# BichenWuUCB/squeezeDet

Hardware: NVIDIA H100
Metric: images/sec (1242x375, b=20) (higher is better)
Workload: dtype f32 (3xTF32 wgmma, fp32 accumulate)

## Files before the change

squeezedet_b200/csrc/conv_pool_simt.cu:

```cuda
#include <math_constants.h>

#include "common.cuh"

namespace sqdet {
namespace {

constexpr int PT_H = 4, PT_W = 16;
constexpr int CT_H = 2 * PT_H + 1, CT_W = 2 * PT_W + 1;
constexpr int CT_PIX = CT_H * CT_W;
constexpr int PIX_PER_THREAD = (CT_PIX + 63) / 64;

struct ConvPoolParams {
  const float* x;
  const float* w;
  const float* bias;
  const float* scale;
  const float* shift;
  float* y;
  int B, H, W, Cout;
  int Hc, Wc;
  int Hp, Wp;
  int cpad_t, cpad_l;
  int ppad_t, ppad_l;
  int relu;
  int tiles_w, tiles_h;
};

template <int KS, int NT, int MINB>
__global__ void __launch_bounds__(NT, MINB)
conv_pool_simt_kernel(const ConvPoolParams p) {
  constexpr int PH = 2 * (CT_H - 1) + KS;
  constexpr int PW = 2 * (CT_W - 1) + KS;
  constexpr int K = KS * KS * 3;
  extern __shared__ __align__(16) float sm[];
  float* s_patch = sm;
  float* s_w = s_patch + ((PH * PW * 3 + 3) & ~3);
  float* s_conv = s_w + K * p.Cout;

  const int tid = threadIdx.x;
  const int nthreads = blockDim.x;
  int tile = blockIdx.x;
  const int tw = tile % p.tiles_w;
  tile /= p.tiles_w;
  const int th = tile % p.tiles_h;
  const int img = tile / p.tiles_h;
  const int ph0 = th * PT_H, pw0 = tw * PT_W;
  const int ch0 = 2 * ph0 - p.ppad_t, cw0 = 2 * pw0 - p.ppad_l;
  const int iy0 = 2 * ch0 - p.cpad_t, ix0 = 2 * cw0 - p.cpad_l;

  for (int i = tid; i < K * p.Cout / 4; i += nthreads) {
    const unsigned dst = (unsigned)__cvta_generic_to_shared(s_w + i * 4);
    asm volatile("cp.async.cg.shared.global [%0], [%1], 16;" ::"r"(dst), "l"(p.w + i * 4) : "memory");
  }
  {
    const float* xin = p.x + (size_t)img * p.H * p.W * 3;
    const int wid = tid >> 5, lane = tid & 31, nwarps = nthreads >> 5;
    for (int row = wid; row < PH; row += nwarps) {
      const int iy = iy0 + row;
      const bool row_ok = iy >= 0 && iy < p.H;
      const float* src = xin + (size_t)(row_ok ? iy : 0) * p.W * 3;
#pragma unroll
      for (int it = 0; it < (PW * 3 + 31) / 32; ++it) {
        const int col = lane + it * 32;
        if (col < PW * 3) {
          const int ixc = ix0 * 3 + col;
          const bool ok = row_ok && ixc >= 0 && ixc < p.W * 3;
          const unsigned dst = (unsigned)__cvta_generic_to_shared(s_patch + row * (PW * 3) + col);
          const int nbytes = ok ? 4 : 0;
          asm volatile("cp.async.ca.shared.global [%0], [%1], 4, %2;" ::"r"(dst),
                       "l"(src + (ok ? ixc : 0)), "r"(nbytes)
                       : "memory");
        }
      }
    }
  }
  asm volatile("cp.async.commit_group;" ::: "memory");
  asm volatile("cp.async.wait_group 0;" ::: "memory");
  __syncthreads();

  const int cg = tid >> 6;
  const int l64 = tid & 63;
  float acc[PIX_PER_THREAD][16];
#pragma unroll
  for (int i = 0; i < PIX_PER_THREAD; ++i)
#pragma unroll
    for (int c = 0; c < 16; ++c) acc[i][c] = 0.f;
  int pbase[PIX_PER_THREAD];
#pragma unroll
  for (int i = 0; i < PIX_PER_THREAD; ++i) {
    int px = l64 + 64 * i;
    if (px >= CT_PIX) px = CT_PIX - 1;
    const int cr = px / CT_W, cc = px - cr * CT_W;
    pbase[i] = (2 * cr * PW + 2 * cc) * 3;
  }
  const float* wg = s_w + cg * 16;
  for (int a = 0; a < KS; ++a) {
#pragma unroll
    for (int bc = 0; bc < KS * 3; ++bc) {
      const int k = a * KS * 3 + bc;
      float xx[PIX_PER_THREAD];
#pragma unroll
      for (int i = 0; i < PIX_PER_THREAD; ++i) xx[i] = s_patch[pbase[i] + a * PW * 3 + bc];
#pragma unroll
      for (int q = 0; q < 4; ++q) {
        const float4 w4 = *reinterpret_cast<const float4*>(wg + k * p.Cout + q * 4);
        const float wv[4] = {w4.x, w4.y, w4.z, w4.w};
#pragma unroll
        for (int i = 0; i < PIX_PER_THREAD; ++i)
#pragma unroll
          for (int c = 0; c < 4; ++c) acc[i][q * 4 + c] = fmaf(xx[i], wv[c], acc[i][q * 4 + c]);
      }
    }
  }

  {
    float bv[16], sv[16], hv[16];
#pragma unroll
    for (int c = 0; c < 16; ++c) {
      bv[c] = p.bias ? __ldg(p.bias + cg * 16 + c) : 0.f;
      sv[c] = p.scale ? __ldg(p.scale + cg * 16 + c) : 1.f;
      hv[c] = p.scale ? __ldg(p.shift + cg * 16 + c) : 0.f;
    }
    float* tile_c = s_conv + (size_t)cg * CT_PIX * 16;
#pragma unroll
    for (int i = 0; i < PIX_PER_THREAD; ++i) {
      const int px = l64 + 64 * i;
      if (px < CT_PIX) {
        const int cr = px / CT_W, cc = px - cr * CT_W;
        const int oh = ch0 + cr, ow = cw0 + cc;
        const bool ok = oh >= 0 && oh < p.Hc && ow >= 0 && ow < p.Wc;
        const int sw = (px >> 1) & 3;
#pragma unroll
        for (int j = 0; j < 4; ++j) {
          float o[4];
#pragma unroll
          for (int e = 0; e < 4; ++e) {
            float f = acc[i][j * 4 + e] + bv[j * 4 + e];
            if (p.scale) f = f * sv[j * 4 + e] + hv[j * 4 + e];
            if (p.relu) f = fmaxf(f, 0.f);
            o[e] = ok ? f : -CUDART_INF_F;
          }
          *reinterpret_cast<float4*>(tile_c + px * 16 + ((j ^ sw) << 2)) =
              make_float4(o[0], o[1], o[2], o[3]);
        }
      }
    }
  }
  __syncthreads();

  const int chunks = p.Cout / 4;
  for (int u = tid; u < PT_H * PT_W * chunks; u += nthreads) {
    const int chunk = u % chunks, pp = u / chunks;
    const int py = pp / PT_W, pxp = pp - py * PT_W;
    const int ph = ph0 + py, pw = pw0 + pxp;
    if (ph >= p.Hp || pw >= p.Wp) continue;
    const int g = chunk >> 2, j = chunk & 3;
    const float* tile_c = s_conv + (size_t)g * CT_PIX * 16;
    float4 m = make_float4(-CUDART_INF_F, -CUDART_INF_F, -CUDART_INF_F, -CUDART_INF_F);
#pragma unroll
    for (int a = 0; a < 3; ++a)
#pragma unroll
      for (int b = 0; b < 3; ++b) {
        const int px = (2 * py + a) * CT_W + 2 * pxp + b;
        const float4 q = *reinterpret_cast<const float4*>(tile_c + px * 16 + ((j ^ ((px >> 1) & 3)) << 2));
        m.x = fmaxf(m.x, q.x); m.y = fmaxf(m.y, q.y);
        m.z = fmaxf(m.z, q.z); m.w = fmaxf(m.w, q.w);
      }
    *reinterpret_cast<float4*>(p.y + (((size_t)img * p.Hp + ph) * p.Wp + pw) * p.Cout + chunk * 4) = m;
  }
}

template <int KS>
size_t smem_bytes_for(int Cout) {
  constexpr int PH = 2 * (CT_H - 1) + KS, PW = 2 * (CT_W - 1) + KS;
  return sizeof(float) * ((size_t)((PH * PW * 3 + 3) & ~3) + (size_t)KS * KS * 3 * Cout +
                          (size_t)(Cout / 16) * CT_PIX * 16);
}

void (*const kConvPoolKernels[4])(ConvPoolParams) = {
    conv_pool_simt_kernel<3, 256, 2>, conv_pool_simt_kernel<3, 384, 1>,
    conv_pool_simt_kernel<7, 256, 1>, conv_pool_simt_kernel<7, 384, 1>};

int conv_pool_instance(int ksize, int threads) { return (ksize == 7 ? 2 : 0) + (threads > 256); }

}

bool conv_pool_simt_eligible(int Cin, int Cout, int ksize, int stride, int pool_size,
                             int pool_stride) {
  return Cin == 3 && (ksize == 3 || ksize == 7) && stride == 2 && pool_size == 3 &&
         pool_stride == 2 && Cout % 16 == 0 && Cout >= 16 && Cout <= 96;
}

int launch_conv_pool_simt(const float* x, const float* w, const float* bias, const float* scale,
                          const float* shift, float* y, int B, int H, int W, int Cout, int ksize,
                          int conv_padding, int relu, int pool_padding, cudaStream_t stream) {
  if (!conv_pool_simt_eligible(3, Cout, ksize, 2, 3, 2))
    return fail(SQDET_ERR_UNSUPPORTED, "conv+pool fusion: unsupported shape");
  const Geom ch = tf_geometry(H, ksize, 2, conv_padding), cw = tf_geometry(W, ksize, 2, conv_padding);
  if (ch.out <= 0 || cw.out <= 0) return fail(SQDET_ERR_INVALID_ARG, "conv+pool: empty conv output");
  const Geom ph = tf_geometry(ch.out, 3, 2, pool_padding), pw = tf_geometry(cw.out, 3, 2, pool_padding);
  if (ph.out <= 0 || pw.out <= 0) return fail(SQDET_ERR_INVALID_ARG, "conv+pool: empty pooled output");
  ConvPoolParams p;
  p.x = x; p.w = w; p.bias = bias; p.scale = scale; p.shift = shift; p.y = y;
  p.B = B; p.H = H; p.W = W; p.Cout = Cout;
  p.Hc = ch.out; p.Wc = cw.out; p.Hp = ph.out; p.Wp = pw.out;
  p.cpad_t = ch.pad_before; p.cpad_l = cw.pad_before;
  p.ppad_t = ph.pad_before; p.ppad_l = pw.pad_before;
  p.relu = relu;
  p.tiles_h = (p.Hp + PT_H - 1) / PT_H;
  p.tiles_w = (p.Wp + PT_W - 1) / PT_W;
  const unsigned grid = (unsigned)(B * p.tiles_h * p.tiles_w);
  const int threads = 64 * (Cout / 16);
  const size_t smem = ksize == 3 ? smem_bytes_for<3>(Cout) : smem_bytes_for<7>(Cout);
  if (smem > 232448) return fail(SQDET_ERR_UNSUPPORTED, "conv+pool: tile does not fit in smem");
  const int inst = conv_pool_instance(ksize, threads);
  static unsigned long long attr_devs[4] = {};
  int dev = 0;
  SQ_CUDA(cudaGetDevice(&dev));
  if (dev >= 64 || !((attr_devs[inst] >> dev) & 1ull)) {
    SQ_CUDA(cudaFuncSetAttribute(kConvPoolKernels[inst], cudaFuncAttributeMaxDynamicSharedMemorySize,
                                 232448));
    if (dev < 64) attr_devs[inst] |= 1ull << dev;
  }
  kConvPoolKernels[inst]<<<grid, threads, smem, stream>>>(p);
  SQ_CHECK_LAUNCH("conv_pool_simt_kernel");
  return SQDET_OK;
}

}
```

Measured before the change: 4265.

## Make fused conv+pool kernel persistent with double-buffered patch prefetch

Turns the stem conv+maxpool kernel into a persistent grid sized by occupancy. Each block loads the weights and affine parameters once, then loops over tiles while prefetching the next input patch into a second buffer with cp.async. The patch is also split into even and odd columns and the weights regrouped per channel group, to reduce shared-memory bank conflicts for the stride-2 reads. Pooling reuses row maxima down each column. In exchange it uses more shared memory, which may lower occupancy, and the single-tile-per-block parallelism becomes a fixed grid.

After: 4319 (median of 6 runs). +1.3%, better.

```diff
diff --git a/squeezedet_b200/csrc/conv_pool_simt.cu b/squeezedet_b200/csrc/conv_pool_simt.cu
--- a/squeezedet_b200/csrc/conv_pool_simt.cu
+++ b/squeezedet_b200/csrc/conv_pool_simt.cu
@@ -26,155 +26,209 @@
   int tiles_w, tiles_h;
 };
 
+template <int KS>
+struct Patch {
+  static constexpr int H = 2 * (CT_H - 1) + KS;
+  static constexpr int W = 2 * (CT_W - 1) + KS;
+  static constexpr int HALF = (W + 1) / 2 * 3;
+  static constexpr int ROW = 2 * HALF;
+  static constexpr int FLOATS = (H * ROW + 3) & ~3;
+};
+
+__device__ __forceinline__ void cp_async4(float* dst, const float* src, bool ok) {
+  const unsigned d = (unsigned)__cvta_generic_to_shared(dst);
+  asm volatile("cp.async.ca.shared.global [%0], [%1], 4, %2;" ::"r"(d), "l"(src), "r"(ok ? 4 : 0)
+               : "memory");
+}
+
+template <int KS>
+__device__ __forceinline__ void load_patch(const ConvPoolParams& p, int tile, float* s_patch) {
+  using P = Patch<KS>;
+  const int tw = tile % p.tiles_w;
+  const int t2 = tile / p.tiles_w;
+  const int th = t2 % p.tiles_h;
+  const int img = t2 / p.tiles_h;
+  const int iy0 = 2 * (2 * th * PT_H - p.ppad_t) - p.cpad_t;
+  const int ix0 = 2 * (2 * tw * PT_W - p.ppad_l) - p.cpad_l;
+  const float* xin = p.x + (size_t)img * p.H * p.W * 3;
+  const int wid = threadIdx.x >> 5, lane = threadIdx.x & 31, nwarps = blockDim.x >> 5;
+  for (int row = wid; row < P::H; row += nwarps) {
+    const int iy = iy0 + row;
+    const bool row_ok = iy >= 0 && iy < p.H;
+    const float* src = xin + (size_t)(row_ok ? iy : 0) * p.W * 3;
+    float* dst = s_patch + row * P::ROW;
+#pragma unroll 1
+    for (int px = lane; px < P::W; px += 32) {
+      const int ix = ix0 + px;
+      const bool ok = row_ok && ix >= 0 && ix < p.W;
+      const float* s = src + (ok ? ix * 3 : 0);
+      float* d = dst + (px & 1) * P::HALF + (px >> 1) * 3;
+      cp_async4(d, s, ok);
+      cp_async4(d + 1, s + 1, ok);
+      cp_async4(d + 2, s + 2, ok);
+    }
+  }
+}
+
 template <int KS, int NT, int MINB>
 __global__ void __launch_bounds__(NT, MINB)
 conv_pool_simt_kernel(const ConvPoolParams p) {
-  constexpr int PH = 2 * (CT_H - 1) + KS;
-  constexpr int PW = 2 * (CT_W - 1) + KS;
+  using P = Patch<KS>;
   constexpr int K = KS * KS * 3;
   extern __shared__ __align__(16) float sm[];
   float* s_patch = sm;
-  float* s_w = s_patch + ((PH * PW * 3 + 3) & ~3);
-  float* s_conv = s_w + K * p.Cout;
+  float* s_w = s_patch + 2 * P::FLOATS;
+  float* s_aff = s_w + K * p.Cout;
+  float* s_conv = s_aff + 3 * p.Cout;
 
   const int tid = threadIdx.x;
   const int nthreads = blockDim.x;
-  int tile = blockIdx.x;
-  const int tw = tile % p.tiles_w;
-  tile /= p.tiles_w;
-  const int th = tile % p.tiles_h;
-  const int img = tile / p.tiles_h;
-  const int ph0 = th * PT_H, pw0 = tw * PT_W;
-  const int ch0 = 2 * ph0 - p.ppad_t, cw0 = 2 * pw0 - p.ppad_l;
-  const int iy0 = 2 * ch0 - p.cpad_t, ix0 = 2 * cw0 - p.cpad_l;
+  const int ntiles = p.B * p.tiles_h * p.tiles_w;
 
   for (int i = tid; i < K * p.Cout / 4; i += nthreads) {
-    const unsigned dst = (unsigned)__cvta_generic_to_shared(s_w + i * 4);
+    const int k = i / (p.Cout / 4), r = i - k * (p.Cout / 4);
+    const unsigned dst = (unsigned)__cvta_generic_to_shared(s_w + ((r >> 2) * K + k) * 16 + (r & 3) * 4);
     asm volatile("cp.async.cg.shared.global [%0], [%1], 16;" ::"r"(dst), "l"(p.w + i * 4) : "memory");
   }
-  {
-    const float* xin = p.x + (size_t)img * p.H * p.W * 3;
-    const int wid = tid >> 5, lane = tid & 31, nwarps = nthreads >> 5;
-    for (int row = wid; row < PH; row += nwarps) {
-      const int iy = iy0 + row;
-      const bool row_ok = iy >= 0 && iy < p.H;
-      const float* src = xin + (size_t)(row_ok ? iy : 0) * p.W * 3;
-#pragma unroll
-      for (int it = 0; it < (PW * 3 + 31) / 32; ++it) {
-        const int col = lane + it * 32;
-        if (col < PW * 3) {
-          const int ixc = ix0 * 3 + col;
-          const bool ok = row_ok && ixc >= 0 && ixc < p.W * 3;
-          const unsigned dst = (unsigned)__cvta_generic_to_shared(s_patch + row * (PW * 3) + col);
-          const int nbytes = ok ? 4 : 0;
-          asm volatile("cp.async.ca.shared.global [%0], [%1], 4, %2;" ::"r"(dst),
-                       "l"(src + (ok ? ixc : 0)), "r"(nbytes)
-                       : "memory");
+  for (int c = tid; c < p.Cout; c += nthreads) {
+    s_aff[c] = p.bias ? __ldg(p.bias + c) : 0.f;
+    s_aff[p.Cout + c] = p.scale ? __ldg(p.scale + c) : 1.f;
+    s_aff[2 * p.Cout + c] = p.scale ? __ldg(p.shift + c) : 0.f;
+  }
+  if ((int)blockIdx.x < ntiles) load_patch<KS>(p, blockIdx.x, s_patch);
+  asm volatile("cp.async.commit_group;" ::: "memory");
+
+  const int cg = tid >> 6;
+  const int l64 = tid & 63;
+  const float* wg = s_w + cg * K * 16;
+  const float* aff = s_aff + cg * 16;
+  float* tile_c = s_conv + (size_t)cg * CT_PIX * 16;
+
+  int buf = 0;
+  for (int tile = blockIdx.x; tile < ntiles; tile += gridDim.x, buf ^= 1) {
+    const int next = tile + gridDim.x;
+    if (next < ntiles) load_patch<KS>(p, next, s_patch + (buf ^ 1) * P::FLOATS);
+    asm volatile("cp.async.commit_group;" ::: "memory");
+    asm volatile("cp.async.wait_group 1;" ::: "memory");
+    __syncthreads();
+
+    const int tw = tile % p.tiles_w;
+    const int t2 = tile / p.tiles_w;
+    const int th = t2 % p.tiles_h;
+    const int img = t2 / p.tiles_h;
+    const int ph0 = th * PT_H, pw0 = tw * PT_W;
+    const int ch0 = 2 * ph0 - p.ppad_t, cw0 = 2 * pw0 - p.ppad_l;
+
+    const float* patch = s_patch + buf * P::FLOATS;
+    float acc[PIX_PER_THREAD][16];
+#pragma unroll
+    for (int i = 0; i < PIX_PER_THREAD; ++i)
+#pragma unroll
+      for (int c = 0; c < 16; ++c) acc[i][c] = 0.f;
+    int pbase[PIX_PER_THREAD];
+#pragma unroll
+    for (int i = 0; i < PIX_PER_THREAD; ++i) {
+      int px = l64 + 64 * i;
+      if (px >= CT_PIX) px = CT_PIX - 1;
+      const int cr = px / CT_W, cc = px - cr * CT_W;
+      pbase[i] = 2 * cr * P::ROW + cc * 3;
+    }
+#pragma unroll (KS == 3 ? 3 : 1)
+    for (int a = 0; a < KS; ++a) {
+#pragma unroll
+      for (int bc = 0; bc < KS * 3; ++bc) {
+        const int b = bc / 3, c = bc - b * 3;
+        const int k = a * KS * 3 + bc;
+        const int off = a * P::ROW + (b & 1) * P::HALF + (b >> 1) * 3 + c;
+        float xx[PIX_PER_THREAD];
+#pragma unroll
+        for (int i = 0; i < PIX_PER_THREAD; ++i) xx[i] = patch[pbase[i] + off];
+#pragma unroll
+        for (int q = 0; q < 4; ++q) {
+          const float4 w4 = *reinterpret_cast<const float4*>(wg + k * 16 + q * 4);
+          const float wv[4] = {w4.x, w4.y, w4.z, w4.w};
+#pragma unroll
+          for (int i = 0; i < PIX_PER_THREAD; ++i)
+#pragma unroll
+            for (int e = 0; e < 4; ++e) acc[i][q * 4 + e] = fmaf(xx[i], wv[e], acc[i][q * 4 + e]);
         }
       }
     }
-  }
-  asm volatile("cp.async.commit_group;" ::: "memory");
-  asm volatile("cp.async.wait_group 0;" ::: "memory");
-  __syncthreads();
-
-  const int cg = tid >> 6;
-  const int l64 = tid & 63;
-  float acc[PIX_PER_THREAD][16];
-#pragma unroll
-  for (int i = 0; i < PIX_PER_THREAD; ++i)
-#pragma unroll
-    for (int c = 0; c < 16; ++c) acc[i][c] = 0.f;
-  int pbase[PIX_PER_THREAD];
-#pragma unroll
-  for (int i = 0; i < PIX_PER_THREAD; ++i) {
-    int px = l64 + 64 * i;
-    if (px >= CT_PIX) px = CT_PIX - 1;
-    const int cr = px / CT_W, cc = px - cr * CT_W;
-    pbase[i] = (2 * cr * PW + 2 * cc) * 3;
-  }
-  const float* wg = s_w + cg * 16;
-  for (int a = 0; a < KS; ++a) {
-#pragma unroll
-    for (int bc = 0; bc < KS * 3; ++bc) {
-      const int k = a * KS * 3 + bc;
-      float xx[PIX_PER_THREAD];
-#pragma unroll
-      for (int i = 0; i < PIX_PER_THREAD; ++i) xx[i] = s_patch[pbase[i] + a * PW * 3 + bc];
-#pragma unroll
-      for (int q = 0; q < 4; ++q) {
-        const float4 w4 = *reinterpret_cast<const float4*>(wg + k * p.Cout + q * 4);
-        const float wv[4] = {w4.x, w4.y, w4.z, w4.w};
-#pragma unroll
-        for (int i = 0; i < PIX_PER_THREAD; ++i)
-#pragma unroll
-          for (int c = 0; c < 4; ++c) acc[i][q * 4 + c] = fmaf(xx[i], wv[c], acc[i][q * 4 + c]);
-      }
-    }
-  }
-
-  {
-    float bv[16], sv[16], hv[16];
-#pragma unroll
-    for (int c = 0; c < 16; ++c) {
-      bv[c] = p.bias ? __ldg(p.bias + cg * 16 + c) : 0.f;
-      sv[c] = p.scale ? __ldg(p.scale + cg * 16 + c) : 1.f;
-      hv[c] = p.scale ? __ldg(p.shift + cg * 16 + c) : 0.f;
-    }
-    float* tile_c = s_conv + (size_t)cg * CT_PIX * 16;
-#pragma unroll
-    for (int i = 0; i < PIX_PER_THREAD; ++i) {
-      const int px = l64 + 64 * i;
-      if (px < CT_PIX) {
-        const int cr = px / CT_W, cc = px - cr * CT_W;
-        const int oh = ch0 + cr, ow = cw0 + cc;
-        const bool ok = oh >= 0 && oh < p.Hc && ow >= 0 && ow < p.Wc;
-        const int sw = (px >> 1) & 3;
-#pragma unroll
-        for (int j = 0; j < 4; ++j) {
+
+#pragma unroll
+    for (int j = 0; j < 4; ++j) {
+      const float4 bv = *reinterpret_cast<const float4*>(aff + j * 4);
+      const float4 sv = *reinterpret_cast<const float4*>(aff + p.Cout + j * 4);
+      const float4 hv = *reinterpret_cast<const float4*>(aff + 2 * p.Cout + j * 4);
+      const float b4[4] = {bv.x, bv.y, bv.z, bv.w};
+      const float s4[4] = {sv.x, sv.y, sv.z, sv.w};
+      const float h4[4] = {hv.x, hv.y, hv.z, hv.w};
+#pragma unroll
+      for (int i = 0; i < PIX_PER_THREAD; ++i) {
+        const int px = l64 + 64 * i;
+        if (px < CT_PIX) {
+          const int cr = px / CT_W, cc = px - cr * CT_W;
+          const int oh = ch0 + cr, ow = cw0 + cc;
+          const bool ok = oh >= 0 && oh < p.Hc && ow >= 0 && ow < p.Wc;
           float o[4];
 #pragma unroll
           for (int e = 0; e < 4; ++e) {
-            float f = acc[i][j * 4 + e] + bv[j * 4 + e];
-            if (p.scale) f = f * sv[j * 4 + e] + hv[j * 4 + e];
+            float f = acc[i][j * 4 + e] + b4[e];
+            if (p.scale) f = f * s4[e] + h4[e];
             if (p.relu) f = fmaxf(f, 0.f);
             o[e] = ok ? f : -CUDART_INF_F;
           }
-          *reinterpret_cast<float4*>(tile_c + px * 16 + ((j ^ sw) << 2)) =
+          *reinterpret_cast<float4*>(tile_c + px * 16 + ((j ^ ((px >> 1) & 3)) << 2)) =
               make_float4(o[0], o[1], o[2], o[3]);
         }
       }
     }
-  }
-  __syncthreads();
-
-  const int chunks = p.Cout / 4;
-  for (int u = tid; u < PT_H * PT_W * chunks; u += nthreads) {
-    const int chunk = u % chunks, pp = u / chunks;
-    const int py = pp / PT_W, pxp = pp - py * PT_W;
-    const int ph = ph0 + py, pw = pw0 + pxp;
-    if (ph >= p.Hp || pw >= p.Wp) continue;
-    const int g = chunk >> 2, j = chunk & 3;
-    const float* tile_c = s_conv + (size_t)g * CT_PIX * 16;
-    float4 m = make_float4(-CUDART_INF_F, -CUDART_INF_F, -CUDART_INF_F, -CUDART_INF_F);
-#pragma unroll
-    for (int a = 0; a < 3; ++a)
-#pragma unroll
-      for (int b = 0; b < 3; ++b) {
-        const int px = (2 * py + a) * CT_W + 2 * pxp + b;
-        const float4 q = *reinterpret_cast<const float4*>(tile_c + px * 16 + ((j ^ ((px >> 1) & 3)) << 2));
-        m.x = fmaxf(m.x, q.x); m.y = fmaxf(m.y, q.y);
-        m.z = fmaxf(m.z, q.z); m.w = fmaxf(m.w, q.w);
+    __syncthreads();
+
+    const int chunks = p.Cout / 4;
+    const int pchunk = tid % chunks, pcol = tid / chunks;
+    const float* pool_c = s_conv + (size_t)(pchunk >> 2) * CT_PIX * 16;
+    const int pw = pw0 + pcol;
+    if (pw < p.Wp) {
+      const int j = pchunk & 3;
+      auto row_max = [&](int r) {
+        float4 m;
+#pragma unroll
+        for (int b = 0; b < 3; ++b) {
+          const int px = r * CT_W + 2 * pcol + b;
+          const float4 q =
+              *reinterpret_cast<const float4*>(pool_c + px * 16 + ((j ^ ((px >> 1) & 3)) << 2));
+          if (b == 0) {
+            m = q;
+          } else {
+            m.x = fmaxf(m.x, q.x); m.y = fmaxf(m.y, q.y);
+            m.z = fmaxf(m.z, q.z); m.w = fmaxf(m.w, q.w);
+          }
+        }
+        return m;
+      };
+      float4 top = row_max(0);
+#pragma unroll 1
+      for (int py = 0; py < PT_H; ++py) {
+        const float4 mid = row_max(2 * py + 1), bot = row_max(2 * py + 2);
+        float4 m;
+        m.x = fmaxf(fmaxf(top.x, mid.x), bot.x); m.y = fmaxf(fmaxf(top.y, mid.y), bot.y);
+        m.z = fmaxf(fmaxf(top.z, mid.z), bot.z); m.w = fmaxf(fmaxf(top.w, mid.w), bot.w);
+        const int ph = ph0 + py;
+        if (ph < p.Hp)
+          *reinterpret_cast<float4*>(p.y + (((size_t)img * p.Hp + ph) * p.Wp + pw) * p.Cout +
+                                     pchunk * 4) = m;
+        top = bot;
       }
-    *reinterpret_cast<float4*>(p.y + (((size_t)img * p.Hp + ph) * p.Wp + pw) * p.Cout + chunk * 4) = m;
-  }
+    }
+  }
+  asm volatile("cp.async.wait_group 0;" ::: "memory");
 }
 
 template <int KS>
 size_t smem_bytes_for(int Cout) {
-  constexpr int PH = 2 * (CT_H - 1) + KS, PW = 2 * (CT_W - 1) + KS;
-  return sizeof(float) * ((size_t)((PH * PW * 3 + 3) & ~3) + (size_t)KS * KS * 3 * Cout +
-                          (size_t)(Cout / 16) * CT_PIX * 16);
+  return sizeof(float) * ((size_t)2 * Patch<KS>::FLOATS + (size_t)KS * KS * 3 * Cout +
+                          (size_t)3 * Cout + (size_t)(Cout / 16) * CT_PIX * 16);
 }
 
 void (*const kConvPoolKernels[4])(ConvPoolParams) = {
@@ -209,19 +263,26 @@
   p.relu = relu;
   p.tiles_h = (p.Hp + PT_H - 1) / PT_H;
   p.tiles_w = (p.Wp + PT_W - 1) / PT_W;
-  const unsigned grid = (unsigned)(B * p.tiles_h * p.tiles_w);
   const int threads = 64 * (Cout / 16);
   const size_t smem = ksize == 3 ? smem_bytes_for<3>(Cout) : smem_bytes_for<7>(Cout);
   if (smem > 232448) return fail(SQDET_ERR_UNSUPPORTED, "conv+pool: tile does not fit in smem");
   const int inst = conv_pool_instance(ksize, threads);
-  static unsigned long long attr_devs[4] = {};
+  static int resident[64][2][6] = {};
   int dev = 0;
   SQ_CUDA(cudaGetDevice(&dev));
-  if (dev >= 64 || !((attr_devs[inst] >> dev) & 1ull)) {
+  int fresh = 0;
+  int* slot = dev < 64 ? &resident[dev][ksize == 7][Cout / 16 - 1] : &fresh;
+  if (*slot == 0) {
     SQ_CUDA(cudaFuncSetAttribute(kConvPoolKernels[inst], cudaFuncAttributeMaxDynamicSharedMemorySize,
                                  232448));
-    if (dev < 64) attr_devs[inst] |= 1ull << dev;
-  }
+    int occ = 0, sms = 0;
+    SQ_CUDA(cudaOccupancyMaxActiveBlocksPerMultiprocessor(&occ, kConvPoolKernels[inst], threads, smem));
+    SQ_CUDA(cudaDeviceGetAttribute(&sms, cudaDevAttrMultiProcessorCount, dev));
+    if (occ < 1) return fail(SQDET_ERR_UNSUPPORTED, "conv+pool: kernel does not fit on an SM");
+    *slot = occ * sms;
+  }
+  const long long tiles = (long long)B * p.tiles_h * p.tiles_w;
+  const unsigned grid = (unsigned)(tiles < *slot ? tiles : *slot);
   kConvPoolKernels[inst]<<<grid, threads, smem, stream>>>(p);
   SQ_CHECK_LAUNCH("conv_pool_simt_kernel");
   return SQDET_OK;
```
